# zju3dv/pvnet

Hardware: NVIDIA H100
Metric: images/sec (480x640, K=9) backbone+vote (higher is better)
Workload: dtype tf32 (fp32 storage, fp32 accumulate; vote fp32/fp64)

## Files before the change

### pvnet_b200/csrc/conv_col.cu

```cuda
#include "conv_tc.cuh"
#include "ptx.cuh"

#include <cstdlib>
#include <mutex>
#include <new>

namespace pvnet {

int g_conv_mode = 0;

namespace {

constexpr int COL_TH = 16, COL_TW = 8;
constexpr int COL_THREADS = 384;
constexpr int HEAD_MAX = 64;

__host__ __device__ constexpr int head_pitch(int hc) { return hc <= 8 ? 8 : (hc <= 24 ? 24 : 40); }
constexpr int HEAD_CPITCH = COL_TH * COL_TW + 4;
__host__ __device__ constexpr int head_stage_floats(int hc)
{
    return COL_TH * COL_TW * head_pitch(hc) > hc * HEAD_CPITCH ? COL_TH * COL_TW * head_pitch(hc) : hc * HEAD_CPITCH;
}
__host__ __device__ constexpr int head_stage_bytes(int hc) { return (head_stage_floats(hc) * 4 + COL_TH * COL_TW + 127) & ~127; }

struct ColGeom {
    int Ho, Wo, tiles_x, tiles_y, total_tiles;
    int cin_chunks, cin_pad;
    int split_chunk;
    int pad_l, pad_t;
    int stages;
    int resident;
    int out_cs, out_co, res_cs, res_co;
    int act, round_out;
    int head_cout, head_seg, mask_esz;
    int head_nhwc;
};

__device__ __forceinline__ void head_store_tile(const ColGeom &g, uint32_t sv, uint32_t sm, float *head_out, void *mask,
                                                int img, int y0, int x0, int tid, int nthr)
{
    const int hc = g.head_cout, pp = head_pitch(hc);
    const int nx = min(COL_TW, g.Wo - x0), ny = min(COL_TH, g.Ho - y0);
    const size_t npix = (size_t)g.Ho * g.Wo;
    const bool vec = (reinterpret_cast<uintptr_t>(head_out) & 15) == 0 && (g.head_nhwc ? hc % 4 == 0 : g.Wo % 4 == 0);
    for (int u = tid; u < 32 * hc; u += nthr) {
        if (g.head_nhwc) {
            const int r = u / (2 * hc), e0 = 4 * (u - r * 2 * hc);
            if (r >= ny) continue;
            float *dst = head_out + (((size_t)img * g.Ho + y0 + r) * g.Wo + x0) * hc + e0;
            if (vec) {
                const int col = e0 / hc;
                if (col < nx)
                    *reinterpret_cast<float4 *>(dst) = ptx::lds128(sv + 4u * (uint32_t)((r * COL_TW + col) * pp + e0 - col * hc));
            } else {
#pragma unroll
                for (int i = 0; i < 4; ++i) {
                    const int col = (e0 + i) / hc;
                    if (col < nx) dst[i] = ptx::lds32(sv + 4u * (uint32_t)((r * COL_TW + col) * pp + e0 + i - col * hc));
                }
            }
        } else {
            const int co = u >> 5, r = (u >> 1) & 15, xo = 4 * (u & 1);
            if (r >= ny) continue;
            float *dst = head_out + ((size_t)img * hc + co) * npix + (size_t)(y0 + r) * g.Wo + x0 + xo;
            const uint32_t src = sv + 4u * (uint32_t)(co * HEAD_CPITCH + r * COL_TW + xo);
            if (vec) {
                if (xo < nx) *reinterpret_cast<float4 *>(dst) = ptx::lds128(src);
            } else {
#pragma unroll
                for (int i = 0; i < 4; ++i)
                    if (xo + i < nx) dst[i] = ptx::lds32(src + 4u * i);
            }
        }
    }
    if (!mask) return;
    for (int p = tid; p < COL_TH * COL_TW; p += nthr) {
        const int r = p / COL_TW, c = p % COL_TW;
        if (r >= ny || c >= nx) continue;
        const size_t pix = ((size_t)img * g.Ho + y0 + r) * g.Wo + x0 + c;
        const uint32_t v = ptx::lds8(sm + (uint32_t)p);
        if (g.mask_esz == 8) reinterpret_cast<long long *>(mask)[pix] = v;
        else reinterpret_cast<unsigned char *>(mask)[pix] = (unsigned char)v;
    }
}
// ... 11 lines not shown
    static_assert((KC == 16) == (KH == 4), "16-channel chunks are the 4x4 stem's, and only its");
    static_assert(!WIDE || (HEAD && KC == 8 && KH == 3), "wide first source: convraw.0 form only");
    constexpr int ROWB = KC * 4;
    constexpr int B_TILE = BN * ROWB;
    constexpr int PITCH = COL_TW + KH - 1;
    constexpr int A_BOX = (COL_TH + KH - 1) * PITCH * ROWB;
    constexpr int A_BYTES = (A_BOX + 1023) & ~1023;
    constexpr int WIDE_BOX = (COL_TH + KH - 1) * PITCH * 128;
    constexpr int WIDE_BYTES = (WIDE_BOX + 1023) & ~1023;
    extern __shared__ uint8_t smem_raw[];
    uint8_t *smem = reinterpret_cast<uint8_t *>((reinterpret_cast<uintptr_t>(smem_raw) + 1023) & ~uintptr_t(1023));
    const int n_btiles = KH * KH * g.cin_chunks;
    const int n_loads = WIDE ? 2 : g.cin_chunks;
    const int stage_bytes = WIDE ? WIDE_BYTES : A_BYTES + (g.resident ? 0 : KH * KH * B_TILE);
    uint8_t *sB = smem;
    uint8_t *sA = smem + (g.resident ? (size_t)n_btiles * B_TILE : 0);
    uint8_t *sH = sA + (size_t)g.stages * stage_bytes;
    uint8_t *sHS = sH + (HEAD ? 4096 : 0);
    const int hs_bytes = HEAD ? head_stage_bytes(g.head_cout) : 0;
    uint64_t *wfull = reinterpret_cast<uint64_t *>(sHS + 2 * hs_bytes);
    uint64_t *full = wfull + 1;
    uint64_t *empty = full + g.stages;
    uint64_t *hstaged = empty + g.stages;
    uint64_t *hfree = hstaged + 2;
    float *s_bias = reinterpret_cast<float *>(empty + g.stages + (HEAD ? 4 : 0));
    float *s_head = s_bias + 64;
    constexpr int STORE_THREADS = 96;

    const int warp = threadIdx.x >> 5, lane = threadIdx.x & 31;
    if (threadIdx.x == 0) {
        ptx::mbar_init(wfull, 1);
        for (int s = 0; s < g.stages; ++s) {
            ptx::mbar_init(&full[s], 1);
            ptx::mbar_init(&empty[s], 8);
        }
        if (HEAD)
            for (int b = 0; b < 2; ++b) {
                ptx::mbar_init(&hstaged[b], 256);
                ptx::mbar_init(&hfree[b], STORE_THREADS);
            }
        ptx::fence_barrier_init();
    }
    for (int i = threadIdx.x; i < BN; i += blockDim.x) s_bias[i] = bias[i];
    if (HEAD) {
        for (int i = threadIdx.x; i < 32; i += blockDim.x) s_head[i] = i < g.head_cout ? head_b[i] : 0.f;
        for (int i = threadIdx.x; i < 32 * 32; i += blockDim.x) {
            const int n = i >> 5, p = i & 31, q = p & 7;
            const int k = (p & ~7) + (q < 4 ? 2 * q : 2 * (q - 4) + 1);
            const float v = n < g.head_cout ? head_w[n * 32 + k] : 0.f;
            *reinterpret_cast<float *>(sH + ptx::swizzle_off((uint32_t)(n * 128 + p * 4), 128)) = v;
        }
        ptx::fence_proxy_async();
    }
    __syncthreads();
    const int tiles_per_img = g.tiles_x * g.tiles_y;

    if (warp >= 8) {
        const int pw = warp - 8;
        if (pw == 0 && lane == 0 && g.resident) {
            ptx::mbar_arrive_expect_tx(wfull, (uint32_t)(n_btiles * B_TILE));
            for (int cc = WIDE ? g.split_chunk : 0; cc < g.cin_chunks; ++cc)
                for (int t = 0; t < KH * KH; ++t)
                    ptx::tma_load_2d(sB + (size_t)(cc * KH * KH + t) * B_TILE, &tmB, wfull, t * g.cin_pad + cc * KC, 0);
            if (WIDE)
                for (int t = 0; t < KH * KH; ++t) ptx::tma_load_2d(sB + (size_t)t * BN * 128, &tmBw, wfull, t * g.cin_pad, 0);
        }
        if (HEAD && pw != 0) {
            const int tid = threadIdx.x - 9 * 32;
            int it = 0;
            for (int tile = blockIdx.x; tile < g.total_tiles; tile += gridDim.x, ++it) {
                const int b = it & 1;
// ... 19 lines not shown
            const int y0 = tyi * COL_TH, x0 = txi * COL_TW;
            for (int cc = 0; cc < n_loads; ++cc) {
                uint8_t *st = sA + (size_t)s * stage_bytes;
                if (WIDE) {
                    if (pw == 0 && lane == 0) {
                        ptx::mbar_wait(&empty[s], ph ^ 1u);
                        ptx::mbar_arrive_expect_tx(&full[s], (uint32_t)(cc == 0 ? WIDE_BOX : A_BOX));
                        ptx::tma_load_4d(st, cc == 0 ? &tmA : &tmA2, &full[s], 0, x0 - g.pad_l, y0 - g.pad_t, img);
                    }
                    __syncwarp();
                } else if (pw == 0) {
                    if (lane == 0) {
                        ptx::mbar_wait(&empty[s], ph ^ 1u);
                        ptx::mbar_arrive_expect_tx(&full[s], tx_bytes);
                        if (cc < g.split_chunk)
                            ptx::tma_load_4d(st, &tmA, &full[s], cc * KC, x0 - g.pad_l, y0 - g.pad_t, img);
                        else
                            ptx::tma_load_4d(st, &tmA2, &full[s], (cc - g.split_chunk) * KC, x0 - g.pad_l, y0 - g.pad_t, img);
                        if (!g.resident)
                            for (int t = 0; t < KH * KH; ++t)
                                ptx::tma_load_2d(st + A_BYTES + (size_t)t * B_TILE, &tmB, &full[s], t * g.cin_pad + cc * KC, 0);
                    }
                    __syncwarp();
                }
                if (++s == g.stages) {
                    s = 0;
                    ph ^= 1u;
                }
            }
        }
        return;
    }

    const int wg = warp >> 2, wq = warp & 3;
    const int g8 = lane >> 2, t4 = lane & 3;
    const uint32_t sA_u = ptx::smem_u32(sA), sB_u = ptx::smem_u32(sB);
    if (g.resident) ptx::mbar_wait(wfull, 0);
    int s = 0;
    uint32_t ph = 0;
    int it = 0;
    for (int tile = blockIdx.x; tile < g.total_tiles; tile += gridDim.x, ++it) {
        float acc[BN / 2];
#pragma unroll
        for (int i = 0; i < BN / 2; ++i) acc[i] = 0.f;
        int prev = -1;
        for (int cc = 0; cc < n_loads; ++cc) {
            ptx::mbar_wait(&full[s], ph);
            const uint32_t a0 = sA_u + (uint32_t)s * (uint32_t)stage_bytes;
            ptx::wgmma_fence();
            if (WIDE && cc == 0) {
                const uint64_t ad0 = ptx::make_kmajor_desc(a0 + (uint32_t)(8 * wg * PITCH * 128), 128, PITCH * 128);
                const uint64_t bd0 = ptx::make_kmajor_desc(sB_u, 128);
#pragma unroll
                for (int ks = 0; ks < 4; ++ks)
#pragma unroll
                    for (int t = 0; t < KH * KH; ++t)
                        ptx::Wgmma<BN>::ss(acc, ad0 + (uint64_t)(((t / KH) * PITCH + t % KH) * 128 / 16 + 2 * ks),
                                           bd0 + (uint64_t)(t * (BN * 128) / 16 + 2 * ks), (t | ks) != 0 ? 1u : 0u);
            } else {
                const int c8 = WIDE ? g.split_chunk : cc;
                const uint32_t b0 = g.resident ? sB_u + (uint32_t)(c8 * KH * KH * B_TILE) : a0 + (uint32_t)A_BYTES;
                const uint64_t ad0 = ptx::make_kmajor_desc(a0 + (uint32_t)(8 * wg * PITCH * ROWB), ROWB, PITCH * ROWB);
                const uint64_t bd0 = ptx::make_kmajor_desc(b0, ROWB);
#pragma unroll
                for (int t = 0; t < KH * KH; ++t) {
                    const uint64_t ad = ad0 + (uint64_t)(((t / KH) * PITCH + t % KH) * ROWB / 16);
                    const uint64_t bd = bd0 + (uint64_t)(t * B_TILE / 16);
#pragma unroll
                    for (int ks = 0; ks < KC / 8; ++ks)
                        ptx::Wgmma<BN>::ss(acc, ad + (uint64_t)(2 * ks), bd + (uint64_t)(2 * ks), (c8 | t | ks) != 0 ? 1u : 0u);
                }
            }
            ptx::wgmma_commit();
            ptx::wgmma_wait<1>();
            ptx::fence_regs(acc);
            if (prev >= 0 && lane == 0) ptx::mbar_arrive(&empty[prev]);
            prev = s;
            if (++s == g.stages) {
                s = 0;
                ph ^= 1u;
            }
        }
        ptx::wgmma_wait<0>();
        ptx::fence_regs(acc);
        if (lane == 0) ptx::mbar_arrive(&empty[prev]);

        const int img = tile / tiles_per_img;
        const int trem = tile - img * tiles_per_img;
        const int tyi = trem / g.tiles_x, txi = trem - tyi * g.tiles_x;
        const int ty = 8 * wg + 2 * wq;
        if constexpr (!HEAD) {
            bool ok[2];
            size_t pix[2];
#pragma unroll
            for (int h = 0; h < 2; ++h) {
                const int y = tyi * COL_TH + ty + h, x = txi * COL_TW + g8;
                ok[h] = y < g.Ho && x < g.Wo;
                pix[h] = ok[h] ? ((size_t)img * g.Ho + y) * g.Wo + x : 0;
            }
            float2 rv[2][BN / 8];
            if (res) {
#pragma unroll
                for (int h = 0; h < 2; ++h)
#pragma unroll
                    for (int j = 0; j < BN / 8; ++j)
                        rv[h][j] = ok[h] ? __ldg(reinterpret_cast<const float2 *>(res + pix[h] * g.res_cs + g.res_co + 8 * j + 2 * t4))
                                         : make_float2(0.f, 0.f);
            }
#pragma unroll
            for (int h = 0; h < 2; ++h) {
                if (!ok[h]) continue;
                float *optr = out + pix[h] * g.out_cs + g.out_co;
#pragma unroll
                for (int j = 0; j < BN / 8; ++j) {
                    const int c = 8 * j + 2 * t4;
                    float2 v = make_float2(acc[4 * j + 2 * h] + s_bias[c], acc[4 * j + 2 * h + 1] + s_bias[c + 1]);
                    if (res) {
                        v.x += rv[h][j].x;
                        v.y += rv[h][j].y;
                    }
                    v.x = epi_act(v.x, g.act, g.round_out);
                    v.y = epi_act(v.y, g.act, g.round_out);
                    *reinterpret_cast<float2 *>(optr + c) = v;
                }
            }
        } else {
            uint32_t a2[4][4];
#pragma unroll
            for (int j = 0; j < 4; ++j)
#pragma unroll
                for (int f = 0; f < 4; ++f) {
                    const int r = 4 * j + ((f & 1) << 1) + (f >> 1);
                    const int c = 8 * j + 2 * t4 + (f >> 1);
                    a2[j][f] = __float_as_uint(ptx::round_tf32(epi_act(acc[r] + s_bias[c], g.act, g.round_out)));
                }
            float hacc[16];
#pragma unroll
            for (int i = 0; i < 16; ++i) hacc[i] = 0.f;
            const uint64_t hd = ptx::make_kmajor_desc(ptx::smem_u32(sH), 128);
            ptx::wgmma_fence();
#pragma unroll
            for (int j = 0; j < 4; ++j) ptx::Wgmma<32>::rs(hacc, a2[j], hd + (uint64_t)(2 * j), j != 0 ? 1u : 0u);
            ptx::wgmma_commit();
            ptx::wgmma_wait<0>();
            ptx::fence_regs(hacc);
            const int hc = g.head_cout, pp = head_pitch(hc);
            const uint32_t sv = ptx::smem_u32(sHS) + (uint32_t)((it & 1) * hs_bytes);
            const uint32_t sm = sv + 4u * (uint32_t)head_stage_floats(hc);
            ptx::mbar_wait(&hfree[it & 1], ((uint32_t)(it >> 1) & 1u) ^ 1u);
#pragma unroll
            for (int h = 0; h < 2; ++h) {
                const uint32_t p = (uint32_t)((ty + h) * COL_TW + g8);
                float best = -INFINITY;
                int best_c = 0;
#pragma unroll
                for (int j = 0; j < 4; ++j) {
                    const int co = 8 * j + 2 * t4;
                    float val[2];
#pragma unroll
                    for (int e = 0; e < 2; ++e) {
                        val[e] = hacc[4 * j + 2 * h + e] + s_head[co + e];
                        if (co + e < g.head_seg && val[e] > best) {
                            best = val[e];
                            best_c = co + e;
                        }
                    }
                    if (co < hc) {
                        if (g.head_nhwc) {
                            ptx::sts64(sv + 4u * (p * pp + co), make_float2(val[0], val[1]));
                        } else {
                            ptx::sts32(sv + 4u * (co * HEAD_CPITCH + p), val[0]);
                            if (co + 1 < hc) ptx::sts32(sv + 4u * ((co + 1) * HEAD_CPITCH + p), val[1]);
                        }
                    }
                }
#pragma unroll
                for (int o = 1; o < 4; o <<= 1) {
                    const float ob = __shfl_xor_sync(0xffffffffu, best, o);
                    const int oc = __shfl_xor_sync(0xffffffffu, best_c, o);
                    if (ob > best || (ob == best && oc < best_c)) {
                        best = ob;
                        best_c = oc;
                    }
                }
                if (t4 == 0) ptx::sts8(sm + p, (uint32_t)best_c);
            }
            ptx::mbar_arrive(&hstaged[it & 1]);
        }
    }
}

struct ColPlan {
    CUtensorMap tmA, tmA2, tmB, tmBw;
    ColGeom g;
    int kc, ksize, head, bn, wide;
    unsigned grid;
    size_t smem;
    const float *bias, *res;
    float *out;
    HeadDesc hd;
};

constexpr size_t SMEM_LIMIT = 227 * 1024;

int col_kc(int Cin) { return Cin % 32 == 0 ? 32 : (Cin == 16 ? 16 : 8); }
int col_cin_pad(int Cin) { return Cin == 16 ? 16 : (Cin + 31) / 32 * 32; }

size_t col_smem(int kc, int ksize, int cin_chunks, int bn, int stages, bool head, bool resident)
{
    const size_t rowb = (size_t)kc * 4;
    const size_t a_box = (size_t)(COL_TH + ksize - 1) * (COL_TW + ksize - 1) * rowb;
    const size_t a = (a_box + 1023) & ~(size_t)1023, bt = (size_t)bn * rowb;
    return 1024 + (resident ? (size_t)ksize * ksize * cin_chunks * bt : 0) +
           (size_t)stages * (a + (resident ? 0 : (size_t)ksize * ksize * bt)) + (head ? 4096 : 0) +
           (size_t)(1 + 2 * stages) * 8 + (64 + 32) * 4;
}

template <int KC, bool HEAD, int KH, int BN, bool WIDE = false>
int col_launch(const ColPlan &p, cudaStream_t s)
// ... 161 lines not shown
```

### pvnet_b200/csrc/ptx.cuh

```cuda
#pragma once
#include <cstdint>
#include <cuda.h>
#include <cuda_runtime.h>

namespace ptx {

__device__ __forceinline__ uint32_t smem_u32(const void *p)
{
    return static_cast<uint32_t>(__cvta_generic_to_shared(p));
}

__device__ __forceinline__ bool elect_one()
{
    uint32_t pred = 0;
    asm volatile(
        "{\n\t"
        ".reg .pred P1;\n\t"
        "elect.sync _|P1, 0xffffffff;\n\t"
        "selp.b32 %0, 1, 0, P1;\n\t"
        "}\n"
        : "=r"(pred));
    return pred != 0;
}

// ... 51 lines not shown
    while (!mbar_try_wait(bar, parity)) {
    }
}

__device__ __forceinline__ void prefetch_tensormap(const CUtensorMap *m)
{
    asm volatile("prefetch.tensormap [%0];" ::"l"(reinterpret_cast<uint64_t>(m)) : "memory");
}
__device__ __forceinline__ void tma_load_4d(void *smem_dst, const CUtensorMap *m, uint64_t *bar, int c0, int c1,
                                            int c2, int c3)
{
    asm volatile(
        "cp.async.bulk.tensor.4d.shared::cluster.global.mbarrier::complete_tx::bytes [%0], [%1, {%3, %4, %5, %6}], [%2];"
        ::"r"(smem_u32(smem_dst)), "l"(reinterpret_cast<uint64_t>(m)), "r"(smem_u32(bar)), "r"(c0), "r"(c1), "r"(c2),
        "r"(c3)
        : "memory");
}
__device__ __forceinline__ void tma_load_2d(void *smem_dst, const CUtensorMap *m, uint64_t *bar, int c0, int c1)
{
    asm volatile(
        "cp.async.bulk.tensor.2d.shared::cluster.global.mbarrier::complete_tx::bytes [%0], [%1, {%3, %4}], [%2];"
        ::"r"(smem_u32(smem_dst)), "l"(reinterpret_cast<uint64_t>(m)), "r"(smem_u32(bar)), "r"(c0), "r"(c1)
        : "memory");
}

__device__ __forceinline__ void tma_store_4d(const CUtensorMap *m, const void *smem_src, int c0, int c1, int c2, int c3)
{
    asm volatile("cp.async.bulk.tensor.4d.global.shared::cta.bulk_group [%0, {%2, %3, %4, %5}], [%1];" ::"l"(
                     reinterpret_cast<uint64_t>(m)),
                 "r"(smem_u32(smem_src)), "r"(c0), "r"(c1), "r"(c2), "r"(c3)
                 : "memory");
}
__device__ __forceinline__ void tma_store_commit() { asm volatile("cp.async.bulk.commit_group;" ::: "memory"); }
__device__ __forceinline__ void tma_store_wait_read() { asm volatile("cp.async.bulk.wait_group.read 0;" ::: "memory"); }
__device__ __forceinline__ void tma_store_wait_read1() { asm volatile("cp.async.bulk.wait_group.read 1;" ::: "memory"); }
__device__ __forceinline__ void tma_store_wait_all() { asm volatile("cp.async.bulk.wait_group 0;" ::: "memory"); }
__device__ __forceinline__ void sts128(uint32_t addr, float4 v)
{
    asm volatile("st.shared.v4.f32 [%0], {%1, %2, %3, %4};" ::"r"(addr), "f"(v.x), "f"(v.y), "f"(v.z), "f"(v.w) : "memory");
}
__device__ __forceinline__ float4 lds128(uint32_t addr)
{
    float4 v;
    asm volatile("ld.shared.v4.f32 {%0, %1, %2, %3}, [%4];" : "=f"(v.x), "=f"(v.y), "=f"(v.z), "=f"(v.w) : "r"(addr) : "memory");
    return v;
}
__device__ __forceinline__ void sts64(uint32_t addr, float2 v)
{
    asm volatile("st.shared.v2.f32 [%0], {%1, %2};" ::"r"(addr), "f"(v.x), "f"(v.y) : "memory");
}
__device__ __forceinline__ float2 lds64(uint32_t addr)
{
    float2 v;
    asm volatile("ld.shared.v2.f32 {%0, %1}, [%2];" : "=f"(v.x), "=f"(v.y) : "r"(addr) : "memory");
    return v;
}
__device__ __forceinline__ void sts32(uint32_t addr, float v) { asm volatile("st.shared.f32 [%0], %1;" ::"r"(addr), "f"(v) : "memory"); }
__device__ __forceinline__ float lds32(uint32_t addr)
{
    float v;
    asm volatile("ld.shared.f32 %0, [%1];" : "=f"(v) : "r"(addr) : "memory");
    return v;
}
__device__ __forceinline__ void sts8(uint32_t addr, uint32_t v) { asm volatile("st.shared.u8 [%0], %1;" ::"r"(addr), "r"(v) : "memory"); }
__device__ __forceinline__ uint32_t lds8(uint32_t addr)
{
    uint32_t v;
    asm volatile("ld.shared.u8 %0, [%1];" : "=r"(v) : "r"(addr) : "memory");
    return v;
}
__device__ __forceinline__ void tma_store_4d_u32(const CUtensorMap *m, uint32_t smem_src, int c0, int c1, int c2, int c3)
{
    asm volatile("cp.async.bulk.tensor.4d.global.shared::cta.bulk_group [%0, {%2, %3, %4, %5}], [%1];" ::"l"(
                     reinterpret_cast<uint64_t>(m)),
                 "r"(smem_src), "r"(c0), "r"(c1), "r"(c2), "r"(c3)
                 : "memory");
}
__device__ __forceinline__ void named_bar_sync(int id, int nthreads)
{
    asm volatile("bar.sync %0, %1;" ::"r"(id), "r"(nthreads) : "memory");
}

__device__ __forceinline__ uint32_t cluster_ctarank()
{
    uint32_t r;
    asm volatile("mov.u32 %0, %%cluster_ctarank;" : "=r"(r));
    return r;
}
__device__ __forceinline__ void cluster_sync()
{
    asm volatile("barrier.cluster.arrive.release.aligned;\n\tbarrier.cluster.wait.acquire.aligned;" ::: "memory");
}
__device__ __forceinline__ uint32_t mapa(const void *p, uint32_t rank)
{
    uint32_t r;
    asm volatile("mapa.shared::cluster.u32 %0, %1, %2;" : "=r"(r) : "r"(smem_u32(p)), "r"(rank));
    return r;
}
__device__ __forceinline__ float ld_cluster_f32(uint32_t addr)
{
    float v;
    asm volatile("ld.shared::cluster.f32 %0, [%1];" : "=f"(v) : "r"(addr) : "memory");
    return v;
}
__device__ __forceinline__ unsigned long long ld_cluster_u64(uint32_t addr)
{
    unsigned long long v;
    asm volatile("ld.shared::cluster.u64 %0, [%1];" : "=l"(v) : "r"(addr) : "memory");
    return v;
}

__device__ __forceinline__ void wgmma_fence() { asm volatile("wgmma.fence.sync.aligned;" ::: "memory"); }
__device__ __forceinline__ void wgmma_commit() { asm volatile("wgmma.commit_group.sync.aligned;" ::: "memory"); }
template <int N>
// ... 108 lines not shown
```

### pvnet_b200/csrc/conv_tc.cu

```cuda
#include "conv_tc.cuh"
#include "ptx.cuh"

#include <cstdlib>
#include <mutex>
#include <new>

namespace pvnet {

struct ConvGeom {
    int Ho, Wo;
    int tiles_x, tiles_y, total_m_tiles;
    int TH, TW;
    int taps, cin_chunks, cin_pad;
    int Cout, BN;
    int out_cs, out_co;
    int res_cs, res_co;
    int act;
    int round_out;
    signed char tap_map[9];
    short tap_ox[9], tap_oy[9];
    int n_items;
    int stages;
};

struct AMaps {
    CUtensorMap m[4];
};

constexpr int CONV_THREADS = 288;
constexpr int CONV_KC = 32;
constexpr int CONV_A_BYTES = 128 * CONV_KC * 4;
constexpr int CONV_SLAB = 32;
constexpr int CONV_SLAB_BYTES = 128 * CONV_SLAB * 4;
constexpr int CONV_EPI_BAR = 1;

template <int BN>
__global__ void __launch_bounds__(CONV_THREADS, 1)
    k_conv_tap(const __grid_constant__ AMaps amaps, const __grid_constant__ CUtensorMap tmB,
               const __grid_constant__ CUtensorMap tmOut, const __grid_constant__ CUtensorMap tmRes,
               const __grid_constant__ ConvGeom g, const float *__restrict__ bias, const int has_res)
{
    constexpr int B_BYTES = BN * CONV_KC * 4;
    constexpr int STAGE_BYTES = CONV_A_BYTES + B_BYTES;
    constexpr int SLABS = BN / CONV_SLAB;
    const int STAGES = g.stages;
    extern __shared__ uint8_t smem_raw[];
    uint8_t *smem = reinterpret_cast<uint8_t *>((reinterpret_cast<uintptr_t>(smem_raw) + 1023) & ~uintptr_t(1023));
    uint8_t *slab = smem + (size_t)STAGES * STAGE_BYTES;
    uint64_t *full = reinterpret_cast<uint64_t *>(slab + 2 * CONV_SLAB_BYTES);
    uint64_t *empty = full + STAGES;
    uint64_t *res_full = empty + STAGES;
    uint64_t *res_free = res_full + 2;

    const int warp = threadIdx.x >> 5, lane = threadIdx.x & 31;
    const int tiles_per_img = g.tiles_x * g.tiles_y;
    const int n_tiles_n = g.Cout / BN;
    const int nkb = g.taps * g.cin_chunks;
    const int unit = (int)blockIdx.x, nunits = (int)gridDim.x;
    auto item_tile = [&](int item, int &m_tile, int &n0) {
        m_tile = item / n_tiles_n;
        n0 = (item - m_tile * n_tiles_n) * BN;
    };

    if (threadIdx.x == 0) {
        for (int s = 0; s < STAGES; ++s) {
            ptx::mbar_init(&full[s], 1);
            ptx::mbar_init(&empty[s], 8);
        }
        for (int i = 0; i < 2; ++i) {
            ptx::mbar_init(&res_full[i], 1);
            ptx::mbar_init(&res_free[i], 1);
        }
        ptx::fence_barrier_init();
    }
    __syncthreads();

    if (warp == 8) {
        if (lane == 0) {
            int r_item = has_res ? unit : g.n_items, r_slab = 0;
            uint32_t rq = 0;
            auto poll_res = [&]() {
                if (r_item >= g.n_items) return;
                const uint32_t b = rq & 1u;
                if (!ptx::mbar_test_wait(&res_free[b], ((rq >> 1) & 1u) ^ 1u)) return;
                int m_tile, n0;
                item_tile(r_item, m_tile, n0);
                const int img = m_tile / tiles_per_img;
                const int trem = m_tile - img * tiles_per_img;
                const int tyi = trem / g.tiles_x, txi = trem - tyi * g.tiles_x;
                ptx::mbar_arrive_expect_tx(&res_full[b], (uint32_t)CONV_SLAB_BYTES);
                ptx::tma_load_4d(slab + b * CONV_SLAB_BYTES, &tmRes, &res_full[b], n0 + r_slab * CONV_SLAB, txi * g.TW,
                                 tyi * g.TH, img);
                ++rq;
                if (++r_slab == SLABS) {
                    r_slab = 0;
                    r_item += nunits;
                }
            };
            int s = 0;
            uint32_t ph = 0;
            for (int item = unit; item < g.n_items; item += nunits) {
                int m_tile, n0;
                item_tile(item, m_tile, n0);
                const int img = m_tile / tiles_per_img;
                const int trem = m_tile - img * tiles_per_img;
                const int tyi = trem / g.tiles_x, txi = trem - tyi * g.tiles_x;
                const int y0 = tyi * g.TH, x0 = txi * g.TW;
                for (int tap = 0; tap < g.taps; ++tap)
                    for (int cc = 0; cc < g.cin_chunks; ++cc) {
                        poll_res();
                        while (!(has_res ? ptx::mbar_test_wait(&empty[s], ph ^ 1u) : ptx::mbar_try_wait(&empty[s], ph ^ 1u)))
                            poll_res();
                        ptx::mbar_arrive_expect_tx(&full[s], (uint32_t)STAGE_BYTES);
                        uint8_t *sa = smem + (size_t)s * STAGE_BYTES;
                        ptx::tma_load_4d(sa, &amaps.m[g.tap_map[tap]], &full[s], cc * CONV_KC, x0 + g.tap_ox[tap],
                                         y0 + g.tap_oy[tap], img);
                        ptx::tma_load_2d(sa + CONV_A_BYTES, &tmB, &full[s], tap * g.cin_pad + cc * CONV_KC, n0);
                        if (++s == STAGES) {
                            s = 0;
                            ph ^= 1u;
                        }
                    }
            }
            while (r_item < g.n_items) poll_res();
        }
    } else {
        const int wg = warp >> 2, wq = warp & 3;
        const int g8 = lane >> 2, t4 = lane & 3;
        const uint32_t smem_u = ptx::smem_u32(smem);
        int s = 0;
        uint32_t ph = 0, sq = 0;
        for (int item = unit; item < g.n_items; item += nunits) {
            float acc[BN / 2];
#pragma unroll
            for (int i = 0; i < BN / 2; ++i) acc[i] = 0.f;
            int prev = -1;
            for (int kb = 0; kb < nkb; ++kb) {
                ptx::mbar_wait(&full[s], ph);
                const uint32_t sa = smem_u + (uint32_t)s * (uint32_t)STAGE_BYTES;
                const uint64_t adesc = ptx::make_kmajor_desc(sa + (uint32_t)(wg * 64 * 128), 128);
                const uint64_t bdesc = ptx::make_kmajor_desc(sa + (uint32_t)CONV_A_BYTES, 128);
                ptx::wgmma_fence();
#pragma unroll
                for (int k = 0; k < CONV_KC / 8; ++k)
                    ptx::Wgmma<BN>::ss(acc, adesc + (uint64_t)(2 * k), bdesc + (uint64_t)(2 * k), (kb | k) != 0 ? 1u : 0u);
                ptx::wgmma_commit();
                ptx::wgmma_wait<1>();
                ptx::fence_regs(acc);
                if (prev >= 0 && lane == 0) ptx::mbar_arrive(&empty[prev]);
                prev = s;
                if (++s == STAGES) {
                    s = 0;
                    ph ^= 1u;
                }
            }
            ptx::wgmma_wait<0>();
            ptx::fence_regs(acc);
            if (lane == 0) ptx::mbar_arrive(&empty[prev]);

            int m_tile, n0;
            item_tile(item, m_tile, n0);
            const int img = m_tile / tiles_per_img;
            const int trem = m_tile - img * tiles_per_img;
            const int tyi = trem / g.tiles_x, txi = trem - tyi * g.tiles_x;
            const uint32_t row_off = (uint32_t)((wg * 64 + wq * 16 + g8) * 128 + (t4 & 1) * 8);
            const uint32_t swz = (uint32_t)(((t4 >> 1) ^ g8) << 4);
            const uint32_t slab_u = ptx::smem_u32(slab);
#pragma unroll
            for (int j = 0; j < SLABS; ++j, ++sq) {
                const uint32_t b = sq & 1u;
                const uint32_t base = slab_u + b * (uint32_t)CONV_SLAB_BYTES + row_off;
                float2 bv[4];
#pragma unroll
                for (int jj = 0; jj < 4; ++jj)
                    bv[jj] = __ldg(reinterpret_cast<const float2 *>(bias + n0 + CONV_SLAB * j + 8 * jj + 2 * t4));
                if (has_res) ptx::mbar_wait(&res_full[b], (sq >> 1) & 1u);
                else ptx::named_bar_sync(CONV_EPI_BAR, 256);
#pragma unroll
                for (int jj = 0; jj < 4; ++jj)
#pragma unroll
                    for (int h = 0; h < 2; ++h) {
                        const uint32_t addr = base + (uint32_t)(h * 8 * 128) + (swz ^ (uint32_t)(32 * jj));
                        const int a = 4 * (4 * j + jj) + 2 * h;
                        float2 v = make_float2(acc[a] + bv[jj].x, acc[a + 1] + bv[jj].y);
                        if (has_res) {
                            const float2 r = ptx::lds64(addr);
                            v.x += r.x;
                            v.y += r.y;
                        }
                        v.x = epi_act(v.x, g.act, g.round_out);
                        v.y = epi_act(v.y, g.act, g.round_out);
                        ptx::sts64(addr, v);
                    }
                ptx::fence_proxy_async();
                ptx::named_bar_sync(CONV_EPI_BAR, 256);
                if (threadIdx.x == 0) {
                    ptx::tma_store_4d(&tmOut, slab + b * CONV_SLAB_BYTES, n0 + CONV_SLAB * j, txi * g.TW, tyi * g.TH, img);
                    ptx::tma_store_commit();
                    if (j == SLABS - 1) ptx::tma_store_wait_read();
                    else ptx::tma_store_wait_read1();
                    if (has_res) {
                        if (j > 0) ptx::mbar_arrive(&res_free[b ^ 1u]);
                        if (j == SLABS - 1) ptx::mbar_arrive(&res_free[b]);
                    }
                }
                __syncwarp();
            }
        }
        if (threadIdx.x == 0) ptx::tma_store_wait_all();
    }
}

typedef CUresult (*EncodeTiledFn)(CUtensorMap *, CUtensorMapDataType, cuuint32_t, void *, const cuuint64_t *,
                                  const cuuint64_t *, const cuuint32_t *, const cuuint32_t *, CUtensorMapInterleave,
                                  CUtensorMapSwizzle, CUtensorMapL2promotion, CUtensorMapFloatOOBfill);

static EncodeTiledFn encode_fn()
{
    static EncodeTiledFn fn = nullptr;
    static std::once_flag once;
    std::call_once(once, [] {
        void *p = nullptr;
        cudaDriverEntryPointQueryResult q;
        if (cudaGetDriverEntryPoint("cuTensorMapEncodeTiled", &p, cudaEnableDefault, &q) == cudaSuccess &&
            q == cudaDriverEntryPointSuccess)
            fn = reinterpret_cast<EncodeTiledFn>(p);
    });
    return fn;
}

int tma_encode(CUtensorMap *m, const void *base, int rank, const cuuint64_t *dims, const cuuint64_t *strides_bytes,
               const cuuint32_t *box, int swizzle_bytes)
{
    EncodeTiledFn fn = encode_fn();
    if (!fn) {
        set_error("cuTensorMapEncodeTiled entry point unavailable");
        return PVNET_E_CUDA;
// ... 101 lines not shown
        cuuint64_t dims[4] = {(cuuint64_t)d.Cin, (cuuint64_t)(d.W / d.stride), (cuuint64_t)(d.H / d.stride),
                              (cuuint64_t)d.b};
        cuuint64_t strides[3] = {(cuuint64_t)d.stride * d.in_cs * 4, (cuuint64_t)d.stride * d.W * d.in_cs * 4,
                                 (cuuint64_t)d.H * d.W * d.in_cs * 4};
        cuuint32_t box[4] = {(cuuint32_t)kc, (cuuint32_t)g.TW, (cuuint32_t)g.TH, 1};
        int rc = tma_encode(&p->amaps.m[pl], base, 4, dims, strides, box, swz);
        if (rc) return rc;
    }
    for (int pl = nplanes; pl < 4; ++pl) p->amaps.m[pl] = p->amaps.m[0];
    {
        cuuint64_t dims[2] = {(cuuint64_t)g.taps * g.cin_pad, (cuuint64_t)d.Cout};
        cuuint64_t strides[1] = {(cuuint64_t)g.taps * g.cin_pad * 4};
        cuuint32_t box[2] = {(cuuint32_t)kc, (cuuint32_t)g.BN};
        int rc = tma_encode(&p->tmB, d.w, 2, dims, strides, box, swz);
        if (rc) return rc;
    }
    {
        cuuint64_t dims[4] = {(cuuint64_t)d.Cout, (cuuint64_t)g.Wo, (cuuint64_t)g.Ho, (cuuint64_t)d.b};
        cuuint32_t box[4] = {(cuuint32_t)CONV_SLAB, (cuuint32_t)g.TW, (cuuint32_t)g.TH, 1};
        cuuint64_t ostr[3] = {(cuuint64_t)d.out_cs * 4, (cuuint64_t)g.Wo * d.out_cs * 4,
                              (cuuint64_t)g.Ho * g.Wo * d.out_cs * 4};
        int rc = tma_encode(&p->tmOut, d.out + d.out_co, 4, dims, ostr, box, CONV_SLAB * 4);
        if (rc) return rc;
        p->tmRes = p->tmOut;
        if (d.res) {
            PV_CHECK_ARG((uintptr_t)d.res % 16 == 0, "conv: pointers must be 16-byte aligned");
            cuuint64_t rstr[3] = {(cuuint64_t)d.res_cs * 4, (cuuint64_t)g.Wo * d.res_cs * 4,
                                  (cuuint64_t)g.Ho * g.Wo * d.res_cs * 4};
            rc = tma_encode(&p->tmRes, d.res + d.res_co, 4, dims, rstr, box, CONV_SLAB * 4);
            if (rc) return rc;
        }
    }
    const size_t stage_b = (size_t)CONV_A_BYTES + (size_t)g.BN * kc * 4;
    int st = (int)((227 * 1024 - 1024 - 256 - 2 * CONV_SLAB_BYTES) / stage_b);
    if (st > 8) st = 8;
    g.stages = st;
    p->smem = 1024 + (size_t)st * stage_b + 2 * CONV_SLAB_BYTES + 256;
    g.n_items = g.total_m_tiles * (d.Cout / g.BN);
    long long grid = (long long)sm_count();
    if (grid > g.n_items) grid = g.n_items;
    p->grid = dim3((unsigned)grid);
    p->bias = d.bias;
    p->has_res = d.res != nullptr;
    return PVNET_OK;
}

template <int BN>
int conv_launch_t(const ConvPlan &p, cudaStream_t s)
{
    const cudaError_t attr_err = ensure_max_smem((const void *)k_conv_tap<BN>, 227 * 1024);
    PV_CUDA(attr_err);
    k_conv_tap<BN><<<p.grid, CONV_THREADS, p.smem, s>>>(p.amaps, p.tmB, p.tmOut, p.tmRes, p.g, p.bias, p.has_res);
    PV_LAUNCHED("k_conv_tap");
    return PVNET_OK;
}

int conv_launch(const ConvPlan &p, cudaStream_t s)
{
    if (p.g.BN == 256) return conv_launch_t<256>(p, s);
    if (p.g.BN == 128) return conv_launch_t<128>(p, s);
    if (p.g.BN == 64) return conv_launch_t<64>(p, s);
    return conv_launch_t<32>(p, s);
}

size_t conv_plan_size() { return sizeof(ConvPlan); }
int conv_plan_at(const ConvDesc &d, void *storage) { return conv_plan(d, new (storage) ConvPlan()); }
int conv_launch_at(const void *storage, cudaStream_t s) { return conv_launch(*static_cast<const ConvPlan *>(storage), s); }

}

// ... 29 lines not shown
```

Baseline: 1724.

## Ping-pong consumer warpgroups over whole tiles with named-barrier turn handoff

Each of the two consumer warpgroups now computes a full 16x8 tile (two M=64 halves with two accumulator sets) on alternating tiles, instead of both splitting every tile. Named barriers hand the MMA turn between the groups so one group's epilogue (bias, residual, head GEMM, argmax) overlaps the other's main loop, and the mbarrier arrival counts are halved to match. The head store also replaces integer divisions with float reciprocal multiplies. This doubles accumulator registers per thread, which may cause spills, and the float-based division must stay exact for the index ranges used.

```diff
diff --git a/pvnet_b200/csrc/conv_col.cu b/pvnet_b200/csrc/conv_col.cu
--- a/pvnet_b200/csrc/conv_col.cu
+++ b/pvnet_b200/csrc/conv_col.cu
@@ -43,13 +43,14 @@
     const int nx = min(COL_TW, g.Wo - x0), ny = min(COL_TH, g.Ho - y0);
     const size_t npix = (size_t)g.Ho * g.Wo;
     const bool vec = (reinterpret_cast<uintptr_t>(head_out) & 15) == 0 && (g.head_nhwc ? hc % 4 == 0 : g.Wo % 4 == 0);
+    const float inv_row = 1.f / (float)(2 * hc), inv_hc = 1.f / (float)hc;
     for (int u = tid; u < 32 * hc; u += nthr) {
         if (g.head_nhwc) {
-            const int r = u / (2 * hc), e0 = 4 * (u - r * 2 * hc);
+            const int r = __float2int_rz(((float)u + 0.5f) * inv_row), e0 = 4 * (u - r * 2 * hc);
             if (r >= ny) continue;
             float *dst = head_out + (((size_t)img * g.Ho + y0 + r) * g.Wo + x0) * hc + e0;
             if (vec) {
-                const int col = e0 / hc;
+                const int col = __float2int_rz(((float)e0 + 0.5f) * inv_hc);
                 if (col < nx)
                     *reinterpret_cast<float4 *>(dst) = ptx::lds128(sv + 4u * (uint32_t)((r * COL_TW + col) * pp + e0 - col * hc));
             } else {
@@ -127,11 +128,11 @@
         ptx::mbar_init(wfull, 1);
         for (int s = 0; s < g.stages; ++s) {
             ptx::mbar_init(&full[s], 1);
-            ptx::mbar_init(&empty[s], 8);
+            ptx::mbar_init(&empty[s], 4);
         }
         if (HEAD)
             for (int b = 0; b < 2; ++b) {
-                ptx::mbar_init(&hstaged[b], 256);
+                ptx::mbar_init(&hstaged[b], 128);
                 ptx::mbar_init(&hfree[b], STORE_THREADS);
             }
         ptx::fence_barrier_init();
@@ -217,48 +218,68 @@
         return;
     }
 
+    constexpr int TURN_BAR = 1;
     const int wg = warp >> 2, wq = warp & 3;
     const int g8 = lane >> 2, t4 = lane & 3;
     const uint32_t sA_u = ptx::smem_u32(sA), sB_u = ptx::smem_u32(sB);
     if (g.resident) ptx::mbar_wait(wfull, 0);
+    const int n_tiles = (int)blockIdx.x < g.total_tiles ? (g.total_tiles - 1 - (int)blockIdx.x) / (int)gridDim.x + 1 : 0;
     int s = 0;
     uint32_t ph = 0;
-    int it = 0;
-    for (int tile = blockIdx.x; tile < g.total_tiles; tile += gridDim.x, ++it) {
-        float acc[BN / 2];
-#pragma unroll
-        for (int i = 0; i < BN / 2; ++i) acc[i] = 0.f;
+    for (int it = 0; it < n_tiles; ++it) {
+        if ((it & 1) != wg) {
+            for (int i = 0; i < n_loads; ++i)
+                if (++s == g.stages) {
+                    s = 0;
+                    ph ^= 1u;
+                }
+            continue;
+        }
+        const int tile = (int)blockIdx.x + it * (int)gridDim.x;
+        if (it > 0) ptx::named_bar_sync(TURN_BAR + wg, 256);
+        float acc[2][BN / 2];
+#pragma unroll
+        for (int hf = 0; hf < 2; ++hf)
+#pragma unroll
+            for (int i = 0; i < BN / 2; ++i) acc[hf][i] = 0.f;
         int prev = -1;
         for (int cc = 0; cc < n_loads; ++cc) {
             ptx::mbar_wait(&full[s], ph);
             const uint32_t a0 = sA_u + (uint32_t)s * (uint32_t)stage_bytes;
             ptx::wgmma_fence();
             if (WIDE && cc == 0) {
-                const uint64_t ad0 = ptx::make_kmajor_desc(a0 + (uint32_t)(8 * wg * PITCH * 128), 128, PITCH * 128);
+                const uint64_t ad0 = ptx::make_kmajor_desc(a0, 128, PITCH * 128);
                 const uint64_t bd0 = ptx::make_kmajor_desc(sB_u, 128);
 #pragma unroll
                 for (int ks = 0; ks < 4; ++ks)
 #pragma unroll
                     for (int t = 0; t < KH * KH; ++t)
-                        ptx::Wgmma<BN>::ss(acc, ad0 + (uint64_t)(((t / KH) * PITCH + t % KH) * 128 / 16 + 2 * ks),
-                                           bd0 + (uint64_t)(t * (BN * 128) / 16 + 2 * ks), (t | ks) != 0 ? 1u : 0u);
+#pragma unroll
+                        for (int hf = 0; hf < 2; ++hf)
+                            ptx::Wgmma<BN>::ss(acc[hf],
+                                               ad0 + (uint64_t)(((8 * hf + t / KH) * PITCH + t % KH) * 128 / 16 + 2 * ks),
+                                               bd0 + (uint64_t)(t * (BN * 128) / 16 + 2 * ks), (t | ks) != 0 ? 1u : 0u);
             } else {
                 const int c8 = WIDE ? g.split_chunk : cc;
                 const uint32_t b0 = g.resident ? sB_u + (uint32_t)(c8 * KH * KH * B_TILE) : a0 + (uint32_t)A_BYTES;
-                const uint64_t ad0 = ptx::make_kmajor_desc(a0 + (uint32_t)(8 * wg * PITCH * ROWB), ROWB, PITCH * ROWB);
+                const uint64_t ad0 = ptx::make_kmajor_desc(a0, ROWB, PITCH * ROWB);
                 const uint64_t bd0 = ptx::make_kmajor_desc(b0, ROWB);
 #pragma unroll
                 for (int t = 0; t < KH * KH; ++t) {
-                    const uint64_t ad = ad0 + (uint64_t)(((t / KH) * PITCH + t % KH) * ROWB / 16);
                     const uint64_t bd = bd0 + (uint64_t)(t * B_TILE / 16);
 #pragma unroll
                     for (int ks = 0; ks < KC / 8; ++ks)
-                        ptx::Wgmma<BN>::ss(acc, ad + (uint64_t)(2 * ks), bd + (uint64_t)(2 * ks), (c8 | t | ks) != 0 ? 1u : 0u);
+#pragma unroll
+                        for (int hf = 0; hf < 2; ++hf)
+                            ptx::Wgmma<BN>::ss(acc[hf], ad0 + (uint64_t)(((8 * hf + t / KH) * PITCH + t % KH) * ROWB / 16 + 2 * ks),
+                                               bd + (uint64_t)(2 * ks), (c8 | t | ks) != 0 ? 1u : 0u);
                 }
             }
             ptx::wgmma_commit();
+            if (cc == n_loads - 1 && it + 1 < n_tiles) ptx::named_bar_arrive(TURN_BAR + (wg ^ 1), 256);
             ptx::wgmma_wait<1>();
-            ptx::fence_regs(acc);
+            ptx::fence_regs(acc[0]);
+            ptx::fence_regs(acc[1]);
             if (prev >= 0 && lane == 0) ptx::mbar_arrive(&empty[prev]);
             prev = s;
             if (++s == g.stages) {
@@ -267,109 +288,125 @@
             }
         }
         ptx::wgmma_wait<0>();
-        ptx::fence_regs(acc);
+        ptx::fence_regs(acc[0]);
+        ptx::fence_regs(acc[1]);
         if (lane == 0) ptx::mbar_arrive(&empty[prev]);
 
         const int img = tile / tiles_per_img;
         const int trem = tile - img * tiles_per_img;
         const int tyi = trem / g.tiles_x, txi = trem - tyi * g.tiles_x;
-        const int ty = 8 * wg + 2 * wq;
         if constexpr (!HEAD) {
-            bool ok[2];
-            size_t pix[2];
-#pragma unroll
-            for (int h = 0; h < 2; ++h) {
-                const int y = tyi * COL_TH + ty + h, x = txi * COL_TW + g8;
-                ok[h] = y < g.Ho && x < g.Wo;
-                pix[h] = ok[h] ? ((size_t)img * g.Ho + y) * g.Wo + x : 0;
-            }
-            float2 rv[2][BN / 8];
+            bool ok[2][2];
+            size_t pix[2][2];
+#pragma unroll
+            for (int hf = 0; hf < 2; ++hf)
+#pragma unroll
+                for (int h = 0; h < 2; ++h) {
+                    const int y = tyi * COL_TH + 8 * hf + 2 * wq + h, x = txi * COL_TW + g8;
+                    ok[hf][h] = y < g.Ho && x < g.Wo;
+                    pix[hf][h] = ok[hf][h] ? ((size_t)img * g.Ho + y) * g.Wo + x : 0;
+                }
+            float2 rv[2][2][BN / 8];
             if (res) {
 #pragma unroll
-                for (int h = 0; h < 2; ++h)
-#pragma unroll
-                    for (int j = 0; j < BN / 8; ++j)
-                        rv[h][j] = ok[h] ? __ldg(reinterpret_cast<const float2 *>(res + pix[h] * g.res_cs + g.res_co + 8 * j + 2 * t4))
-                                         : make_float2(0.f, 0.f);
-            }
-#pragma unroll
-            for (int h = 0; h < 2; ++h) {
-                if (!ok[h]) continue;
-                float *optr = out + pix[h] * g.out_cs + g.out_co;
-#pragma unroll
-                for (int j = 0; j < BN / 8; ++j) {
-                    const int c = 8 * j + 2 * t4;
-                    float2 v = make_float2(acc[4 * j + 2 * h] + s_bias[c], acc[4 * j + 2 * h + 1] + s_bias[c + 1]);
-                    if (res) {
-                        v.x += rv[h][j].x;
-                        v.y += rv[h][j].y;
+                for (int hf = 0; hf < 2; ++hf)
+#pragma unroll
+                    for (int h = 0; h < 2; ++h)
+#pragma unroll
+                        for (int j = 0; j < BN / 8; ++j)
+                            rv[hf][h][j] = ok[hf][h] ? __ldg(reinterpret_cast<const float2 *>(res + pix[hf][h] * g.res_cs + g.res_co +
+                                                                                             8 * j + 2 * t4))
+                                                     : make_float2(0.f, 0.f);
+            }
+#pragma unroll
+            for (int hf = 0; hf < 2; ++hf)
+#pragma unroll
+                for (int h = 0; h < 2; ++h) {
+                    if (!ok[hf][h]) continue;
+                    float *optr = out + pix[hf][h] * g.out_cs + g.out_co;
+#pragma unroll
+                    for (int j = 0; j < BN / 8; ++j) {
+                        const int c = 8 * j + 2 * t4;
+                        float2 v = make_float2(acc[hf][4 * j + 2 * h] + s_bias[c], acc[hf][4 * j + 2 * h + 1] + s_bias[c + 1]);
+                        if (res) {
+                            v.x += rv[hf][h][j].x;
+                            v.y += rv[hf][h][j].y;
+                        }
+                        v.x = epi_act(v.x, g.act, g.round_out);
+                        v.y = epi_act(v.y, g.act, g.round_out);
+                        *reinterpret_cast<float2 *>(optr + c) = v;
                     }
-                    v.x = epi_act(v.x, g.act, g.round_out);
-                    v.y = epi_act(v.y, g.act, g.round_out);
-                    *reinterpret_cast<float2 *>(optr + c) = v;
-                }
-            }
+                }
         } else {
-            uint32_t a2[4][4];
-#pragma unroll
-            for (int j = 0; j < 4; ++j)
-#pragma unroll
-                for (int f = 0; f < 4; ++f) {
-                    const int r = 4 * j + ((f & 1) << 1) + (f >> 1);
-                    const int c = 8 * j + 2 * t4 + (f >> 1);
-                    a2[j][f] = __float_as_uint(ptx::round_tf32(epi_act(acc[r] + s_bias[c], g.act, g.round_out)));
-                }
-            float hacc[16];
-#pragma unroll
-            for (int i = 0; i < 16; ++i) hacc[i] = 0.f;
+            uint32_t a2[2][4][4];
+#pragma unroll
+            for (int hf = 0; hf < 2; ++hf)
+#pragma unroll
+                for (int j = 0; j < 4; ++j)
+#pragma unroll
+                    for (int f = 0; f < 4; ++f) {
+                        const int r = 4 * j + ((f & 1) << 1) + (f >> 1);
+                        const int c = 8 * j + 2 * t4 + (f >> 1);
+                        a2[hf][j][f] = __float_as_uint(ptx::round_tf32(epi_act(acc[hf][r] + s_bias[c], g.act, g.round_out)));
+                    }
+            float hacc[2][16];
+#pragma unroll
+            for (int hf = 0; hf < 2; ++hf)
+#pragma unroll
+                for (int i = 0; i < 16; ++i) hacc[hf][i] = 0.f;
             const uint64_t hd = ptx::make_kmajor_desc(ptx::smem_u32(sH), 128);
             ptx::wgmma_fence();
 #pragma unroll
-            for (int j = 0; j < 4; ++j) ptx::Wgmma<32>::rs(hacc, a2[j], hd + (uint64_t)(2 * j), j != 0 ? 1u : 0u);
+            for (int hf = 0; hf < 2; ++hf)
+#pragma unroll
+                for (int j = 0; j < 4; ++j) ptx::Wgmma<32>::rs(hacc[hf], a2[hf][j], hd + (uint64_t)(2 * j), j != 0 ? 1u : 0u);
             ptx::wgmma_commit();
             ptx::wgmma_wait<0>();
-            ptx::fence_regs(hacc);
+            ptx::fence_regs(hacc[0]);
+            ptx::fence_regs(hacc[1]);
             const int hc = g.head_cout, pp = head_pitch(hc);
             const uint32_t sv = ptx::smem_u32(sHS) + (uint32_t)((it & 1) * hs_bytes);
             const uint32_t sm = sv + 4u * (uint32_t)head_stage_floats(hc);
             ptx::mbar_wait(&hfree[it & 1], ((uint32_t)(it >> 1) & 1u) ^ 1u);
 #pragma unroll
-            for (int h = 0; h < 2; ++h) {
-                const uint32_t p = (uint32_t)((ty + h) * COL_TW + g8);
-                float best = -INFINITY;
-                int best_c = 0;
-#pragma unroll
-                for (int j = 0; j < 4; ++j) {
-                    const int co = 8 * j + 2 * t4;
-                    float val[2];
-#pragma unroll
-                    for (int e = 0; e < 2; ++e) {
-                        val[e] = hacc[4 * j + 2 * h + e] + s_head[co + e];
-                        if (co + e < g.head_seg && val[e] > best) {
-                            best = val[e];
-                            best_c = co + e;
+            for (int hf = 0; hf < 2; ++hf)
+#pragma unroll
+                for (int h = 0; h < 2; ++h) {
+                    const uint32_t p = (uint32_t)((8 * hf + 2 * wq + h) * COL_TW + g8);
+                    float best = -INFINITY;
+                    int best_c = 0;
+#pragma unroll
+                    for (int j = 0; j < 4; ++j) {
+                        const int co = 8 * j + 2 * t4;
+                        float val[2];
+#pragma unroll
+                        for (int e = 0; e < 2; ++e) {
+                            val[e] = hacc[hf][4 * j + 2 * h + e] + s_head[co + e];
+                            if (co + e < g.head_seg && val[e] > best) {
+                                best = val[e];
+                                best_c = co + e;
+                            }
+                        }
+                        if (co < hc) {
+                            if (g.head_nhwc) {
+                                ptx::sts64(sv + 4u * (p * pp + co), make_float2(val[0], val[1]));
+                            } else {
+                                ptx::sts32(sv + 4u * (co * HEAD_CPITCH + p), val[0]);
+                                if (co + 1 < hc) ptx::sts32(sv + 4u * ((co + 1) * HEAD_CPITCH + p), val[1]);
+                            }
                         }
                     }
-                    if (co < hc) {
-                        if (g.head_nhwc) {
-                            ptx::sts64(sv + 4u * (p * pp + co), make_float2(val[0], val[1]));
-                        } else {
-                            ptx::sts32(sv + 4u * (co * HEAD_CPITCH + p), val[0]);
-                            if (co + 1 < hc) ptx::sts32(sv + 4u * ((co + 1) * HEAD_CPITCH + p), val[1]);
+#pragma unroll
+                    for (int o = 1; o < 4; o <<= 1) {
+                        const float ob = __shfl_xor_sync(0xffffffffu, best, o);
+                        const int oc = __shfl_xor_sync(0xffffffffu, best_c, o);
+                        if (ob > best || (ob == best && oc < best_c)) {
+                            best = ob;
+                            best_c = oc;
                         }
                     }
-                }
-#pragma unroll
-                for (int o = 1; o < 4; o <<= 1) {
-                    const float ob = __shfl_xor_sync(0xffffffffu, best, o);
-                    const int oc = __shfl_xor_sync(0xffffffffu, best_c, o);
-                    if (ob > best || (ob == best && oc < best_c)) {
-                        best = ob;
-                        best_c = oc;
-                    }
-                }
-                if (t4 == 0) ptx::sts8(sm + p, (uint32_t)best_c);
-            }
+                    if (t4 == 0) ptx::sts8(sm + p, (uint32_t)best_c);
+                }
             ptx::mbar_arrive(&hstaged[it & 1]);
         }
     }
diff --git a/pvnet_b200/csrc/ptx.cuh b/pvnet_b200/csrc/ptx.cuh
--- a/pvnet_b200/csrc/ptx.cuh
+++ b/pvnet_b200/csrc/ptx.cuh
@@ -155,6 +155,10 @@
 {
     asm volatile("bar.sync %0, %1;" ::"r"(id), "r"(nthreads) : "memory");
 }
+__device__ __forceinline__ void named_bar_arrive(int id, int nthreads)
+{
+    asm volatile("bar.arrive %0, %1;" ::"r"(id), "r"(nthreads) : "memory");
+}
 
 __device__ __forceinline__ uint32_t cluster_ctarank()
 {
```

Result: faster. 1760, median of 6 (+2.1%).

## Decouple residual prefetch buffers from output staging slabs in conv epilogue

Applied to the files above, without the earlier changes.

Residual tiles were previously loaded into the same two smem slabs used for staging the TMA output store, so residual prefetch had to wait for each store to drain. This adds a separate ring of residual buffers, sized from leftover shared memory and possibly trading away one pipeline stage, with 8-warp release barriers. Residual and bias are now added into the accumulators before the staging barrier, and the store-wait per item relaxes to wait_group.read 1. The aim is to let residual loads run ahead of the epilogue and cut serialization between stores and residual reads. The cost is extra smem, which may reduce mainloop stages for residual layers.

```diff
diff --git a/pvnet_b200/csrc/conv_tc.cu b/pvnet_b200/csrc/conv_tc.cu
--- a/pvnet_b200/csrc/conv_tc.cu
+++ b/pvnet_b200/csrc/conv_tc.cu
@@ -21,6 +21,7 @@
     short tap_ox[9], tap_oy[9];
     int n_items;
     int stages;
+    int res_bufs;
 };
 
 struct AMaps {
@@ -43,14 +44,15 @@
     constexpr int B_BYTES = BN * CONV_KC * 4;
     constexpr int STAGE_BYTES = CONV_A_BYTES + B_BYTES;
     constexpr int SLABS = BN / CONV_SLAB;
-    const int STAGES = g.stages;
+    const int STAGES = g.stages, RBUFS = g.res_bufs;
     extern __shared__ uint8_t smem_raw[];
     uint8_t *smem = reinterpret_cast<uint8_t *>((reinterpret_cast<uintptr_t>(smem_raw) + 1023) & ~uintptr_t(1023));
     uint8_t *slab = smem + (size_t)STAGES * STAGE_BYTES;
-    uint64_t *full = reinterpret_cast<uint64_t *>(slab + 2 * CONV_SLAB_BYTES);
+    uint8_t *rslab = slab + 2 * CONV_SLAB_BYTES;
+    uint64_t *full = reinterpret_cast<uint64_t *>(rslab + (size_t)RBUFS * CONV_SLAB_BYTES);
     uint64_t *empty = full + STAGES;
     uint64_t *res_full = empty + STAGES;
-    uint64_t *res_free = res_full + 2;
+    uint64_t *res_free = res_full + RBUFS;
 
     const int warp = threadIdx.x >> 5, lane = threadIdx.x & 31;
     const int tiles_per_img = g.tiles_x * g.tiles_y;
@@ -67,9 +69,9 @@
             ptx::mbar_init(&full[s], 1);
             ptx::mbar_init(&empty[s], 8);
         }
-        for (int i = 0; i < 2; ++i) {
+        for (int i = 0; i < RBUFS; ++i) {
             ptx::mbar_init(&res_full[i], 1);
-            ptx::mbar_init(&res_free[i], 1);
+            ptx::mbar_init(&res_free[i], 8);
         }
         ptx::fence_barrier_init();
     }
@@ -77,21 +79,23 @@
 
     if (warp == 8) {
         if (lane == 0) {
-            int r_item = has_res ? unit : g.n_items, r_slab = 0;
-            uint32_t rq = 0;
+            int r_item = has_res ? unit : g.n_items, r_slab = 0, rb = 0;
+            uint32_t rph = 0;
             auto poll_res = [&]() {
                 if (r_item >= g.n_items) return;
-                const uint32_t b = rq & 1u;
-                if (!ptx::mbar_test_wait(&res_free[b], ((rq >> 1) & 1u) ^ 1u)) return;
+                if (!ptx::mbar_test_wait(&res_free[rb], rph ^ 1u)) return;
                 int m_tile, n0;
                 item_tile(r_item, m_tile, n0);
                 const int img = m_tile / tiles_per_img;
                 const int trem = m_tile - img * tiles_per_img;
                 const int tyi = trem / g.tiles_x, txi = trem - tyi * g.tiles_x;
-                ptx::mbar_arrive_expect_tx(&res_full[b], (uint32_t)CONV_SLAB_BYTES);
-                ptx::tma_load_4d(slab + b * CONV_SLAB_BYTES, &tmRes, &res_full[b], n0 + r_slab * CONV_SLAB, txi * g.TW,
-                                 tyi * g.TH, img);
-                ++rq;
+                ptx::mbar_arrive_expect_tx(&res_full[rb], (uint32_t)CONV_SLAB_BYTES);
+                ptx::tma_load_4d(rslab + rb * CONV_SLAB_BYTES, &tmRes, &res_full[rb], n0 + r_slab * CONV_SLAB,
+                                 txi * g.TW, tyi * g.TH, img);
+                if (++rb == RBUFS) {
+                    rb = 0;
+                    rph ^= 1u;
+                }
                 if (++r_slab == SLABS) {
                     r_slab = 0;
                     r_item += nunits;
@@ -128,8 +132,8 @@
         const int wg = warp >> 2, wq = warp & 3;
         const int g8 = lane >> 2, t4 = lane & 3;
         const uint32_t smem_u = ptx::smem_u32(smem);
-        int s = 0;
-        uint32_t ph = 0, sq = 0;
+        int s = 0, rb = 0;
+        uint32_t ph = 0, sq = 0, rph = 0;
         for (int item = unit; item < g.n_items; item += nunits) {
             float acc[BN / 2];
 #pragma unroll
@@ -165,44 +169,58 @@
             const int tyi = trem / g.tiles_x, txi = trem - tyi * g.tiles_x;
             const uint32_t row_off = (uint32_t)((wg * 64 + wq * 16 + g8) * 128 + (t4 & 1) * 8);
             const uint32_t swz = (uint32_t)(((t4 >> 1) ^ g8) << 4);
-            const uint32_t slab_u = ptx::smem_u32(slab);
+            const uint32_t slab_u = ptx::smem_u32(slab), rslab_u = ptx::smem_u32(rslab);
 #pragma unroll
             for (int j = 0; j < SLABS; ++j, ++sq) {
+                float2 bv[4];
+#pragma unroll
+                for (int jj = 0; jj < 4; ++jj)
+                    bv[jj] = __ldg(reinterpret_cast<const float2 *>(bias + n0 + CONV_SLAB * j + 8 * jj + 2 * t4));
+#pragma unroll
+                for (int jj = 0; jj < 4; ++jj)
+#pragma unroll
+                    for (int h = 0; h < 2; ++h) {
+                        const int a = 4 * (4 * j + jj) + 2 * h;
+                        acc[a] += bv[jj].x;
+                        acc[a + 1] += bv[jj].y;
+                    }
+                if (has_res) {
+                    ptx::mbar_wait(&res_full[rb], rph);
+                    const uint32_t rbase = rslab_u + (uint32_t)rb * (uint32_t)CONV_SLAB_BYTES + row_off;
+#pragma unroll
+                    for (int jj = 0; jj < 4; ++jj)
+#pragma unroll
+                        for (int h = 0; h < 2; ++h) {
+                            const float2 r = ptx::lds64(rbase + (uint32_t)(h * 8 * 128) + (swz ^ (uint32_t)(32 * jj)));
+                            const int a = 4 * (4 * j + jj) + 2 * h;
+                            acc[a] += r.x;
+                            acc[a + 1] += r.y;
+                        }
+                    __syncwarp();
+                    if (lane == 0) ptx::mbar_arrive(&res_free[rb]);
+                    if (++rb == RBUFS) {
+                        rb = 0;
+                        rph ^= 1u;
+                    }
+                }
                 const uint32_t b = sq & 1u;
                 const uint32_t base = slab_u + b * (uint32_t)CONV_SLAB_BYTES + row_off;
-                float2 bv[4];
+                ptx::named_bar_sync(CONV_EPI_BAR, 256);
 #pragma unroll
                 for (int jj = 0; jj < 4; ++jj)
-                    bv[jj] = __ldg(reinterpret_cast<const float2 *>(bias + n0 + CONV_SLAB * j + 8 * jj + 2 * t4));
-                if (has_res) ptx::mbar_wait(&res_full[b], (sq >> 1) & 1u);
-                else ptx::named_bar_sync(CONV_EPI_BAR, 256);
-#pragma unroll
-                for (int jj = 0; jj < 4; ++jj)
 #pragma unroll
                     for (int h = 0; h < 2; ++h) {
-                        const uint32_t addr = base + (uint32_t)(h * 8 * 128) + (swz ^ (uint32_t)(32 * jj));
                         const int a = 4 * (4 * j + jj) + 2 * h;
-                        float2 v = make_float2(acc[a] + bv[jj].x, acc[a + 1] + bv[jj].y);
-                        if (has_res) {
-                            const float2 r = ptx::lds64(addr);
-                            v.x += r.x;
-                            v.y += r.y;
-                        }
-                        v.x = epi_act(v.x, g.act, g.round_out);
-                        v.y = epi_act(v.y, g.act, g.round_out);
-                        ptx::sts64(addr, v);
+                        const float2 v = make_float2(epi_act(acc[a], g.act, g.round_out),
+                                                     epi_act(acc[a + 1], g.act, g.round_out));
+                        ptx::sts64(base + (uint32_t)(h * 8 * 128) + (swz ^ (uint32_t)(32 * jj)), v);
                     }
                 ptx::fence_proxy_async();
                 ptx::named_bar_sync(CONV_EPI_BAR, 256);
                 if (threadIdx.x == 0) {
                     ptx::tma_store_4d(&tmOut, slab + b * CONV_SLAB_BYTES, n0 + CONV_SLAB * j, txi * g.TW, tyi * g.TH, img);
                     ptx::tma_store_commit();
-                    if (j == SLABS - 1) ptx::tma_store_wait_read();
-                    else ptx::tma_store_wait_read1();
-                    if (has_res) {
-                        if (j > 0) ptx::mbar_arrive(&res_free[b ^ 1u]);
-                        if (j == SLABS - 1) ptx::mbar_arrive(&res_free[b]);
-                    }
+                    ptx::tma_store_wait_read1();
                 }
                 __syncwarp();
             }
@@ -370,10 +388,19 @@
         }
     }
     const size_t stage_b = (size_t)CONV_A_BYTES + (size_t)g.BN * kc * 4;
-    int st = (int)((227 * 1024 - 1024 - 256 - 2 * CONV_SLAB_BYTES) / stage_b);
+    const size_t avail = 227 * 1024 - 1024 - 256 - 2 * CONV_SLAB_BYTES;
+    int st = (int)(avail / stage_b);
     if (st > 8) st = 8;
+    int rbufs = 0;
+    if (d.res) {
+        rbufs = (int)((avail - (size_t)(st - 1) * stage_b) / CONV_SLAB_BYTES);
+        if (rbufs > g.BN / CONV_SLAB) rbufs = g.BN / CONV_SLAB;
+        st = (int)((avail - (size_t)rbufs * CONV_SLAB_BYTES) / stage_b);
+        if (st > 8) st = 8;
+    }
     g.stages = st;
-    p->smem = 1024 + (size_t)st * stage_b + 2 * CONV_SLAB_BYTES + 256;
+    g.res_bufs = rbufs;
+    p->smem = 1024 + (size_t)st * stage_b + (size_t)(2 + rbufs) * CONV_SLAB_BYTES + 256;
     g.n_items = g.total_m_tiles * (d.Cout / g.BN);
     long long grid = (long long)sm_count();
     if (grid > g.n_items) grid = g.n_items;
diff --git a/pvnet_b200/csrc/ptx.cuh b/pvnet_b200/csrc/ptx.cuh
--- a/pvnet_b200/csrc/ptx.cuh
+++ b/pvnet_b200/csrc/ptx.cuh
@@ -107,7 +107,6 @@
                  : "memory");
 }
 __device__ __forceinline__ void tma_store_commit() { asm volatile("cp.async.bulk.commit_group;" ::: "memory"); }
-__device__ __forceinline__ void tma_store_wait_read() { asm volatile("cp.async.bulk.wait_group.read 0;" ::: "memory"); }
 __device__ __forceinline__ void tma_store_wait_read1() { asm volatile("cp.async.bulk.wait_group.read 1;" ::: "memory"); }
 __device__ __forceinline__ void tma_store_wait_all() { asm volatile("cp.async.bulk.wait_group 0;" ::: "memory"); }
 __device__ __forceinline__ void sts128(uint32_t addr, float4 v)
```

New measurement: 1728 before, 1775 after, median of 6. 2.7% higher.
